# KC-decoder/Multimodal-Brain-Pattern-Identification_XAI

Hardware: AMD Instinct MI355X
Metric: samples/sec train (multimodal SpectrogramCNN+EEGNet fusion, B=64/GPU, 4x128x256 spectro + 10000x19 EEG) (higher is better)
Workload: dtype bf16

## Files before the change

include/brainxai.h:

```cpp
#ifndef BRAINXAI_H
#define BRAINXAI_H

#include <stddef.h>
#include <stdint.h>

#ifdef __cplusplus
extern "C" {
#endif

#define BX_VERSION 100

enum { BX_F32 = 0, BX_BF16 = 1 };
enum { BX_POOL_MAX = 0, BX_POOL_AVG = 1 };
enum { BX_OK = 0, BX_EINVAL = -1, BX_EDTYPE = -2, BX_EALIGN = -3, BX_EWORKSPACE = -4, BX_EHIP = -5,
       BX_EUNSUPPORTED = -6 };
enum { BX_ALGO_AUTO = 0, BX_ALGO_DIRECT = 1, BX_ALGO_MFMA = 2 };
enum { BX_EPI_RELU = 1, BX_EPI_MASK_BITS = 2 };

typedef void* bxStream;

int bx_version(void);
const char* bx_last_error_string(void);

int bx_nchw_to_nhwc(const float* src, void* dst, int B, int C, int H, int W, int Cp, int dtype, bxStream stream);
// ... 35 lines not shown
} bxWgradPending;
int bx_conv3x3_wgrad_chained(const void* x, const void* dz, float* dw_oihw, float* dbias, int B, int H, int W, int Cin,
                             int Ci_p, int Co, int dtype, int algo, void* workspace, size_t workspace_bytes,
                             bxWgradPending* pending, bxStream stream);
int bx_conv3x3_wgrad_finish(bxWgradPending* pending, bxStream stream);
int bx_conv3x3_carry(const void* x, const float* packed_f32, const void* packed_mfma, const float* bias,
                     const void* relu_mask_src, const void* addend, void* y, int B, int H, int W, int Ci, int Co,
                     int dtype, int flags, int algo, bxWgradPending* pending, bxStream stream);
int bx_conv3x3_carry_many(const void* x, const float* packed_f32, const void* packed_mfma, const float* bias,
                          const void* relu_mask_src, const void* addend, void* y, int B, int H, int W, int Ci, int Co,
                          int dtype, int flags, int algo, bxWgradPending* pending, int npending, bxStream stream);
typedef struct {
  const void* x; const void* dz;
  float* dw; float* db;
  int Cin, Ci_p, Co;
} bxWgradGroupLayer;
int bx_conv3x3_wgrad_group_supported(int n, const int* Ci_p, const int* Co, int W, int dtype);
size_t bx_conv3x3_wgrad_group_workspace(const bxWgradGroupLayer* layers, int n, int B, int H, int W, int dtype);
int bx_conv3x3_wgrad_group(const bxWgradGroupLayer* layers, int n, int B, int H, int W, int dtype, void* workspace,
                           size_t workspace_bytes, bxWgradPending* pending, bxStream stream);
size_t bx_conv3x3_bwd_fused_workspace(int B, int H, int W, int with_w1);
int bx_conv3x3_bwd_fused(const void* dz, const void* xl, const void* packed_flip, void* dzo, const void* x0, float* dw, float* db,
                         float* dw0, float* db0, int B, int H, int W, int Cin0, void* workspace, size_t workspace_bytes,
                         bxWgradPending* pending, bxStream stream);

int bx_profile_next_conv3(void* ev_start, void* ev_stop);

typedef struct {
  int B, H, W;
  int Cin_p;
  int C;
  int pool;
  int training;
  float eps, momentum;
  float dropout_p;
  uint32_t salt;
  int dtype;
  uint32_t* sync;
  void* route;
  int pool_h, pool_w;
} bxTailDesc;
size_t bx_block_tail_route_bytes(const bxTailDesc* d);
#define BX_TAIL_SYNC_WORDS 8192
#define BX_TAIL_SYNC_FWD 0
#define BX_TAIL_SYNC_BWD 4096
size_t bx_block_tail_workspace(const bxTailDesc* d);
int bx_block_tail_fwd(const bxTailDesc* d, const void* y3, const void* x, const float* w1x1, int Cin,
                      const float* b1x1, const float* bn_weight, const float* bn_bias,
                      float* running_mean, float* running_var, int64_t* num_batches_tracked,
                      const uint64_t* seed, void* pooled, void* out, float* save_mean, float* save_invstd,
                      void* workspace, size_t workspace_bytes, bxStream stream);
int bx_set_tree_max_rows(int rows);
int bx_set_tail_fold(int mask);
int bx_block_conv3_tail_fwd(const bxTailDesc* d, const void* y2, const void* w3_mfma, const float* b3, void* y3,
                            const void* x, const float* w1x1, int Cin, const float* b1x1, const float* bn_weight,
                            const float* bn_bias, float* running_mean, float* running_var, int64_t* num_batches_tracked,
                            const uint64_t* seed, void* pooled, void* out, float* save_mean, float* save_invstd,
                            void* workspace, size_t workspace_bytes, bxStream stream);
int bx_block_tail_bwd(const bxTailDesc* d, const void* dout, const void* y3, const void* x, const void* pooled,
                      const float* w1x1, int Cin, const float* bn_weight, const float* save_mean,
                      const float* save_invstd, const uint64_t* seed, void* dz3, void* dx_skip,
                      float* d_bn_weight, float* d_bn_bias, float* d_w1x1, float* d_b1x1,
                      void* workspace, size_t workspace_bytes, bxStream stream);
int bx_relu(const void* x, void* y, size_t n, int dtype, bxStream stream);

int bx_gap_fc_lsm_fwd(const void* feat, const float* w, const float* b, float* gap_out, float* logp,
                      int B, int HW, int C, int N, int dtype, bxStream stream);
int bx_gap_fc_lsm_bwd(const float* dlogp, const float* logp, const float* gap_out, const float* w,
                      void* dfeat, float* dw, float* db, int B, int HW, int C, int N, int dtype, bxStream stream);
int bx_linear_lsm_fwd(const float* x, const float* w, const float* b, float* logp, int B, int K, int N,
                      bxStream stream);
int bx_linear_lsm_bwd(const float* dlogp, const float* logp, const float* x, const float* w, float* dx,
                      float* dw, float* db, int B, int K, int N, bxStream stream);
int bx_fusion_head_fwd(const float* eeg_logp, const float* spec_logp, const float* w1, const float* b1,
                       const float* w2, const float* b2, float* hidden, float* logp, int B, int N, int Hd,
                       bxStream stream);
int bx_fusion_head_bwd(const float* dlogp, const float* logp, const float* hidden, const float* eeg_logp,
                       const float* spec_logp, const float* w1, const float* w2, float* d_eeg_logp,
                       float* d_spec_logp, float* dw1, float* db1, float* dw2, float* db2, int B, int N, int Hd,
                       bxStream stream);
size_t bx_mm_head_workspace(int B, int N, int Hd);
int bx_mm_head_fwd(const void* feat, const float* eeg_feat, const float* fc_w, const float* fc_b, const float* dense_w,
                   const float* dense_b, const float* w1, const float* b1, const float* w2, const float* b2,
                   float* gap_out, float* spec_logp, float* eeg_logp, float* hidden, float* logp, int B, int HW, int C,
                   int K, int N, int Hd, int dtype, bxStream stream);
int bx_mm_head_bwd(const float* dlogp, const float* logp, const float* hidden, const float* spec_logp,
                   const float* eeg_logp, const float* gap, const float* eeg_feat, const float* fc_w,
                   const float* dense_w, const float* w1, const float* w2, void* dfeat, float* d_eeg_feat,
                   float* d_fc_w, float* d_fc_b, float* d_dense_w, float* d_dense_b, float* dw1, float* db1, float* dw2,
                   float* db2, void* workspace, size_t workspace_bytes, int B, int HW, int C, int K, int N, int Hd,
                   int dtype, bxStream stream);
int bx_kldiv_fwd_bwd(const float* logp, const float* target, float* loss, float* dlogp, int B, int N,
                     int reduction, float grad_scale, bxStream stream);

typedef struct {
  int B, Chans, T;
  int F1, D, F2;
  int K1, K2;
  int P1, P2;
  int training;
  float eps, momentum, dropout_p;
  uint32_t salt;
  int dtype;
  int collapse;
  float dropout_p2;
  const float* const* x_slot;
// ... 190 lines not shown
```

multimodal-brain-pattern-identification_xai_amd/_lib.py:

```python
from __future__ import annotations

import ctypes as C
import os

HERE = os.path.dirname(os.path.abspath(__file__))
LIB_PATH = os.path.join(HERE, "libbrainxai.so")

BX_F32, BX_BF16 = 0, 1
BX_POOL_MAX, BX_POOL_AVG = 0, 1
BX_ALGO_AUTO, BX_ALGO_DIRECT, BX_ALGO_MFMA = 0, 1, 2
BX_EPI_RELU = 1
BX_EPI_MASK_BITS = 2
BX_TAIL_SYNC_WORDS = 8192
BX_EEG_CAM_CONV1, BX_EEG_CAM_DEPTHWISE, BX_EEG_CAM_SEPARABLE = 0, 1, 2
BX_CAM_GRADCAM, BX_CAM_GRADCAM_PP, BX_CAM_LAYERCAM = 0, 1, 2
BX_SCORECAM_PROB, BX_SCORECAM_INCREASE = 0, 1

vp, i32, i64, u32, f32, sz = C.c_void_p, C.c_int, C.c_int64, C.c_uint32, C.c_float, C.c_size_t


class TailDesc(C.Structure):
    _fields_ = [("B", i32), ("H", i32), ("W", i32), ("Cin_p", i32), ("C", i32), ("pool", i32), ("training", i32),
                ("eps", f32), ("momentum", f32), ("dropout_p", f32), ("salt", u32), ("dtype", i32), ("sync", vp), ("route", vp),
                ("pool_h", i32), ("pool_w", i32)]
# ... 26 lines not shown

class WgradPending(C.Structure):
    _fields_ = [("partial", vp), ("dw", vp), ("db", vp), ("nsplit", i32), ("Cin", i32), ("Co", i32), ("ma", i32), ("nb", i32),
                ("ztiles", i32), ("nfrag4", i32), ("valid", i32)]


class WgradGroupLayer(C.Structure):
    _fields_ = [("x", vp), ("dz", vp), ("dw", vp), ("db", vp), ("Cin", i32), ("Ci_p", i32), ("Co", i32)]


class PackJob(C.Structure):
    _fields_ = [("w_oihw", vp), ("packed_mfma", vp), ("Cout", i32), ("Cin", i32), ("I_p", i32), ("O_p", i32),
                ("transpose_flip", i32), ("block_begin", i32)]


class EegGrads(C.Structure):
    _fields_ = [(n, vp) for n in ("conv1_w", "bn1_w", "bn1_b", "dw_w", "bn2_w", "bn2_b", "sep_w", "bn3_w", "bn3_b")]


P = C.POINTER
SIGNATURES = {
    "bx_version": (i32, []),
    "bx_last_error_string": (C.c_char_p, []),
    "bx_nchw_to_nhwc": (i32, [vp, vp, i32, i32, i32, i32, i32, i32, vp]),
    "bx_nhwc_to_nchw": (i32, [vp, vp, i32, i32, i32, i32, i32, i32, vp]),
    "bx_conv3x3_pack": (i32, [vp, vp, vp, i32, i32, i32, i32, i32, vp]),
    "bx_conv3x3_packed_mfma_bytes": (sz, [i32, i32]),
    "bx_conv3x3_packed_split_bytes": (sz, [i32, i32]),
    "bx_conv3x3_pack_split": (i32, [vp, vp, i32, i32, i32, i32, i32, vp]),
    "bx_conv3x3_pack_many": (i32, [vp, i32, i32, vp]),
    "bx_conv3x3_pack_many_layout": (i32, [vp, i32, i32, vp, vp, i32, i32, i32, i32, i32, vp]),
    "bx_conv3x3_pack_layout_ex": (i32, [vp, i32, i32, vp, vp, vp, i32, i32, i32, i32, i32, vp]),
    "bx_conv3x3_pair_supported": (i32, [i32, i32, i32, i32]),
    "bx_conv3x3_pair": (i32, [vp] * 9 + [i32] * 7 + [vp]),
    "bx_conv3x3_pack_many_step": (i32, [vp, i32, i32, vp, vp, i32, i32, i32, i32, i32, vp, vp, vp, vp, vp]),
    "bx_scale_dev": (i32, [vp, vp, vp, sz, vp]),
    "bx_abs": (i32, [vp, vp, sz, vp]),
    "bx_conv3x3": (i32, [vp, vp, vp, vp, vp, vp, vp, i32, i32, i32, i32, i32, i32, i32, i32, vp]),
    "bx_conv3x3_carry": (i32, [vp, vp, vp, vp, vp, vp, vp, i32, i32, i32, i32, i32, i32, i32, i32, P(WgradPending), vp]),
    "bx_conv3x3_carry_many": (i32, [vp, vp, vp, vp, vp, vp, vp, i32, i32, i32, i32, i32, i32, i32, i32, P(WgradPending), i32, vp]),
    "bx_conv3x3_wgrad_group_supported": (i32, [i32, P(i32), P(i32), i32, i32]),
    "bx_conv3x3_wgrad_group_workspace": (sz, [P(WgradGroupLayer), i32, i32, i32, i32, i32]),
    "bx_conv3x3_wgrad_group": (i32, [P(WgradGroupLayer), i32, i32, i32, i32, i32, vp, sz, P(WgradPending), vp]),
    "bx_conv3x3_wgrad_workspace": (sz, [i32, i32, i32, i32, i32, i32, i32]),
    "bx_conv3x3_wgrad": (i32, [vp, vp, vp, vp, i32, i32, i32, i32, i32, i32, i32, i32, vp, sz, vp]),
    "bx_conv3x3_wgrad_chained": (i32, [vp, vp, vp, vp, i32, i32, i32, i32, i32, i32, i32, i32, vp, sz, P(WgradPending), vp]),
    "bx_conv3x3_wgrad_finish": (i32, [P(WgradPending), vp]),
    "bx_conv3x3_bwd_fused_workspace": (sz, [i32, i32, i32, i32]),
    "bx_conv3x3_bwd_fused": (i32, [vp] * 9 + [i32] * 4 + [vp, sz, P(WgradPending), vp]),
    "bx_block_tail_workspace": (sz, [P(TailDesc)]),
    "bx_block_tail_fwd": (i32, [P(TailDesc), vp, vp, vp, i32, vp, vp, vp, vp, vp, vp, vp, vp, vp, vp, vp, vp, sz, vp]),
    "bx_set_tree_max_rows": (i32, [i32]),
    "bx_set_tail_fold": (i32, [i32]),
    "bx_block_tail_route_bytes": (sz, [vp]),
    "bx_block_conv3_tail_fwd": (i32, [P(TailDesc), vp, vp, vp, vp, vp, vp, i32, vp, vp, vp, vp, vp, vp, vp, vp, vp, vp, vp, vp, sz, vp]),
    "bx_block_tail_bwd": (i32, [P(TailDesc), vp, vp, vp, vp, vp, i32, vp, vp, vp, vp, vp, vp, vp, vp, vp, vp, vp, sz, vp]),
    "bx_relu": (i32, [vp, vp, sz, i32, vp]),
    "bx_gap_fc_lsm_fwd": (i32, [vp, vp, vp, vp, vp, i32, i32, i32, i32, i32, vp]),
    "bx_gap_fc_lsm_bwd": (i32, [vp, vp, vp, vp, vp, vp, vp, i32, i32, i32, i32, i32, vp]),
    "bx_linear_lsm_fwd": (i32, [vp, vp, vp, vp, i32, i32, i32, vp]),
    "bx_linear_lsm_bwd": (i32, [vp, vp, vp, vp, vp, vp, vp, i32, i32, i32, vp]),
    "bx_fusion_head_fwd": (i32, [vp, vp, vp, vp, vp, vp, vp, vp, i32, i32, i32, vp]),
    "bx_fusion_head_bwd": (i32, [vp] * 13 + [i32, i32, i32, vp]),
    "bx_mm_head_workspace": (sz, [i32, i32, i32]),
    "bx_mm_head_fwd": (i32, [vp] * 15 + [i32] * 7 + [vp]),
    "bx_mm_head_bwd": (i32, [vp] * 22 + [sz] + [i32] * 7 + [vp]),
    "bx_kldiv_fwd_bwd": (i32, [vp, vp, vp, vp, i32, i32, i32, f32, vp]),
    "bx_eeg_saved_bytes": (sz, [P(EegDesc)]),
    "bx_eeg_workspace": (sz, [P(EegDesc)]),
    "bx_eeg_features_fwd": (i32, [P(EegDesc), P(EegParams), vp, vp, vp, vp, vp, sz, vp]),
    "bx_eeg_features_bwd": (i32, [P(EegDesc), P(EegParams), vp, vp, vp, vp, P(EegGrads), vp, vp, sz, vp]),
    "bx_eeg_saved_layout": (i32, [P(EegDesc), P(sz), P(sz)]),
    "bx_eeg_gradcam_workspace": (sz, [P(EegDesc), i32, i32]),
    "bx_eeg_gradcam": (i32, [P(EegDesc), P(EegParams), vp, vp, vp, i32, i32, i32, vp, vp, vp, vp, sz, vp]),
    "bx_eeg_cam_workspace": (sz, [P(EegDesc), i32, i32, i32]),
    "bx_eeg_cam": (i32, [P(EegDesc), P(EegParams), vp, vp, vp, i32, i32, i32, i32, vp, vp, vp, vp, sz, vp]),
    "bx_eeg_deep_saved_bytes": (sz, [P(EegDeepDesc)]),
    "bx_eeg_deep_workspace": (sz, [P(EegDeepDesc)]),
    "bx_eeg_deep_fwd": (i32, [P(EegDeepDesc), P(EegDeepParams), vp, vp, vp, vp, vp, vp, sz, vp]),
    "bx_eeg_deep_bwd": (i32, [P(EegDeepDesc), P(EegDeepParams), vp, vp, vp, vp, vp, P(EegDeepGrads), vp, vp, sz, vp]),
    "bx_attention_workspace": (sz, [i32]),
    "bx_attention_fwd": (i32, [vp] * 10 + [i32, i32, i32, vp]),
    "bx_attention_bwd": (i32, [vp] * 16 + [sz, i32, i32, i32, vp]),
    "bx_gradcam_reduce": (i32, [vp, vp, vp, vp, i32, i32, i32, i32, i32, i32, vp]),
    "bx_gradcam_head": (i32, [vp] * 12 + [i32] * 8 + [vp]),
    "bx_gradcam_head_sweep": (i32, [vp] * 4 + [i32] + [vp] * 8 + [i32] * 11 + [vp]),
    "bx_cam_reduce": (i32, [vp, vp, vp, vp, i32, i32, i32, i32, i32, i32, i32, vp]),
    "bx_cam_head": (i32, [vp] * 12 + [i32] * 9 + [vp]),
    "bx_cam_head_sweep": (i32, [vp] * 4 + [i32] + [vp] * 8 + [i32] * 12 + [vp]),
    "bx_resize_bilinear": (i32, [vp, vp, i32, i32, i32, i32, i32, vp]),
    "bx_saliency_reduce": (i32, [vp, vp, i32, i32, i32, i32, f32, i32, vp]),
    "bx_axpby": (i32, [vp, vp, sz, f32, f32, vp]),
    "bx_mul": (i32, [vp, vp, vp, sz, vp]),
    "bx_ig_interpolate": (i32, [vp, vp, vp, vp, sz, i32, vp]),
    "bx_ig_accumulate": (i32, [vp, vp, vp, sz, i32, vp]),
    "bx_eeg_stack_iir": (i32, [vp, vp, vp, i32, i32, i32, i32, P(C.c_double), P(C.c_double), i32, i32, f32, f32, vp]),
    "bx_eeg_montage_workspace": (sz, [i32, i32, i32, i32]),
    "bx_eeg_montage_stack": (i32, [vp, vp, vp, vp, i32, i32, i32, i32, i32, P(C.c_double), P(C.c_double), i32, P(C.c_double), P(C.c_double),
                                   i32, f32, vp, vp, sz, vp]),
    "bx_spec_preprocess_workspace": (sz, [i32, i32, i32]),
    "bx_spec_preprocess": (i32, [vp, vp, vp, i32, i32, i32, i32, i32, i32, P(C.c_double), P(C.c_double), P(C.c_double), P(C.c_double),
                                 f32, vp, vp, sz, vp]),
    "bx_spec_regions_workspace": (sz, [i32]),
    "bx_spec_regions": (i32, [vp, vp, vp] + [i32] * 7 + [P(C.c_double), i32, P(C.c_double), i32, f32, vp, sz, vp]),
    "bx_adamw_step": (i32, [vp, vp, vp, vp, sz, f32, f32, f32, f32, f32, f32, vp, vp]),
    "bx_adamw_partials": (sz, [sz]),
# ... 66 lines not shown
```

multimodal-brain-pattern-identification_xai_amd/csrc/tail.hip:

```cpp
#include "bx_common.h"

#define TAIL_MAX_GROUPS 128
#define TAIL_MAX_BLOCKS 2048

struct TailGeom {
  int B, H, W, Ho, Wo, C, Cin_p, ncg, slots;
  long long npool;
  float sy, sx;
};

static int tail_ph(const bxTailDesc* d) { return d->pool_h ? d->pool_h : 2; }
static int tail_pw(const bxTailDesc* d) { return d->pool_w ? d->pool_w : 2; }
static bool tail_2x2(const bxTailDesc* d) { return tail_ph(d) == 2 && tail_pw(d) == 2; }

static int make_geom(const bxTailDesc* d, TailGeom* g) {
  if (tail_ph(d) < 1 || tail_pw(d) < 1) return -5;
  g->B = d->B; g->H = d->H; g->W = d->W; g->Ho = d->H / tail_ph(d); g->Wo = d->W / tail_pw(d); g->C = d->C; g->Cin_p = d->Cin_p;
  if (d->B <= 0 || g->Ho <= 0 || g->Wo <= 0) return -1;
  if (d->C % 8 || d->C > 256 || 256 % (d->C / 8)) return -2;
  if (d->Cin_p % 8 || d->Cin_p <= 0) return -3;
  if ((long long)d->B * d->H * d->W * ((d->Cin_p > d->C ? d->Cin_p : d->C) / 8) >= (1ll << 31)) return -4;
  g->ncg = d->C / 8; g->slots = 256 / g->ncg;
  g->npool = (long long)d->B * g->Ho * g->Wo;
  g->sy = (float)d->H / (float)g->Ho; g->sx = (float)d->W / (float)g->Wo;
// ... 151 lines not shown
        ld8(y3, base + ((size_t)r * g.W + (q - r * pw)) * g.C, w[u]);
      }
#pragma unroll
      for (int u = 0; u < 4; ++u)
        if (q0 + u < area)
#pragma unroll
          for (int j = 0; j < 8; ++j) v[j] = pool == BX_POOL_MAX ? fmaxf(v[j], w[u][j]) : v[j] + w[u][j];
    }
    if (pool != BX_POOL_MAX)
#pragma unroll
      for (int j = 0; j < 8; ++j) v[j] = v[j] / (float)area;
    st8(pooled, (size_t)pp * g.C + cg * 8, v);
    if (want_stats) {
#pragma unroll
      for (int j = 0; j < 8; ++j) {
        const float q = round_as(pooled, v[j]);
        acc[0][j] += q; acc[1][j] += q * q;
      }
    }
  }
  if (!want_stats) return;
  pool_stats_publish(acc, lds, partials, g, tree, fin);
}

template <typename T> struct Raw8;
template <> struct Raw8<bf16_t> {
  uint4 r;
  __device__ __forceinline__ void load(const bf16_t* p, size_t i) { r = *reinterpret_cast<const uint4*>(p + i); }
  __device__ __forceinline__ void get(float v[8]) const {
    const uint32_t w[4] = {r.x, r.y, r.z, r.w};
#pragma unroll
    for (int k = 0; k < 4; ++k) { v[2 * k] = __uint_as_float(w[k] << 16); v[2 * k + 1] = __uint_as_float(w[k] & 0xffff0000u); }
  }
};
template <> struct Raw8<float> {
  float4 a, b;
  __device__ __forceinline__ void load(const float* p, size_t i) { a = *reinterpret_cast<const float4*>(p + i); b = *reinterpret_cast<const float4*>(p + i + 4); }
  __device__ __forceinline__ void get(float v[8]) const { v[0] = a.x; v[1] = a.y; v[2] = a.z; v[3] = a.w; v[4] = b.x; v[5] = b.y; v[6] = b.z; v[7] = b.w; }
};

template <typename T>
__device__ __forceinline__ void skip_sample(const T* __restrict__ x, const TailGeom& g, int b, int oy, int ox, int c0, float out[8]) {
  int y0, y1, x0, x1; float ly, lx;
  bilinear_src(oy, g.sy, g.H, y0, y1, ly);
  bilinear_src(ox, g.sx, g.W, x0, x1, lx);
  const float hy = 1.f - ly, hx = 1.f - lx;
  float p00[8], p01[8], p10[8], p11[8];
  const size_t rb = (size_t)b * g.H;
  ld8(x, ((rb + y0) * g.W + x0) * g.Cin_p + c0, p00); ld8(x, ((rb + y0) * g.W + x1) * g.Cin_p + c0, p01);
  ld8(x, ((rb + y1) * g.W + x0) * g.Cin_p + c0, p10); ld8(x, ((rb + y1) * g.W + x1) * g.Cin_p + c0, p11);
#pragma unroll
  for (int j = 0; j < 8; ++j) out[j] = hy * (hx * p00[j] + lx * p01[j]) + ly * (hx * p10[j] + lx * p11[j]);
}

struct TailFwdPro { const float* rows; int nrows; BxBnFinalize fin; };
template <typename T, int RPT>
__global__ __launch_bounds__(256, sizeof(T) == 4 ? 3 : 4) void k_tail_apply(const T* __restrict__ pooled, const T* __restrict__ x, const float* __restrict__ wT,
    int Cin, const float* __restrict__ b1x1, const float* __restrict__ scale, const float* __restrict__ shift,
    const uint64_t* __restrict__ seed, float dropout_p, uint32_t salt, T* __restrict__ out, TailGeom g,
    const float* __restrict__ ev_gamma, const float* __restrict__ ev_beta, const float* __restrict__ ev_rmean,
    const float* __restrict__ ev_rvar, float eps, float* __restrict__ save_mean, float* __restrict__ save_invstd, TailFwdPro pro) {
  extern __shared__ float xs[];
  const int cg = threadIdx.x % g.ncg, slot = threadIdx.x / g.ncg;
  const int xstride = g.Cin_p + 1, nci8 = g.Cin_p / 8;
  const uint64_t sd = (dropout_p > 0.f && seed) ? seed[0] : 0;
  const float inv_keep = dropout_p > 0.f ? 1.f / (1.f - dropout_p) : 1.f;
  float sc[8], sh[8], bb[8];
  if (pro.rows) {
    __shared__ __attribute__((aligned(8))) double sp[BX_ROWS_TOTAL_LDS(2) / 8];
    __shared__ float ssc[2][256];
    bx_rows_total<2>(pro.rows, pro.nrows, g.C, sp);
    if ((int)threadIdx.x < g.C) {
      const int c = threadIdx.x;
      const BxBnFinalize& f = pro.fin;
      float mean, invstd; double unbiased;
      bx_bn_batch_stats(sp[c], sp[g.C + c], f.count, f.eps, mean, invstd, unbiased);
      const float s_ = f.gamma[c] * invstd, h_ = f.beta[c] - mean * s_;
      ssc[0][c] = s_; ssc[1][c] = h_;
      if (blockIdx.x == 0) {
        f.rmean[c] = (1.f - f.momentum) * f.rmean[c] + f.momentum * mean;
        f.rvar[c] = (1.f - f.momentum) * f.rvar[c] + f.momentum * (float)unbiased;
        if (c == 0 && f.nbt) f.nbt[0] += 1;
        f.scale[c] = s_; f.shift[c] = h_; f.save_mean[c] = mean; f.save_invstd[c] = invstd;
      }
    }
    __syncthreads();
#pragma unroll
    for (int j = 0; j < 8; ++j) { sc[j] = ssc[0][cg * 8 + j]; sh[j] = ssc[1][cg * 8 + j]; bb[j] = b1x1[cg * 8 + j]; }
  } else if (ev_gamma) {
#pragma unroll
    for (int j = 0; j < 8; ++j) {
      const int c = cg * 8 + j;
      const float is = 1.0f / sqrtf(ev_rvar[c] + eps), s_ = ev_gamma[c] * is;
      sc[j] = s_; sh[j] = ev_beta[c] - ev_rmean[c] * s_; bb[j] = b1x1[c];
    }
    if (blockIdx.x == 0 && (int)threadIdx.x < g.C) {
      save_mean[threadIdx.x] = ev_rmean[threadIdx.x];
      save_invstd[threadIdx.x] = 1.0f / sqrtf(ev_rvar[threadIdx.x] + eps);
    }
  } else {
#pragma unroll
    for (int j = 0; j < 8; ++j) { sc[j] = scale[cg * 8 + j]; sh[j] = shift[cg * 8 + j]; bb[j] = b1x1[cg * 8 + j]; }
  }
  const long long nsteps = (g.npool + (long long)gridDim.x * g.slots - 1) / ((long long)gridDim.x * g.slots);
  for (long long st = 0; st < nsteps; ++st) {
    const long long p0 = (st * gridDim.x + blockIdx.x) * g.slots;
    Raw8<T> pvr;
    {
      const long long ppq = p0 + slot;
      pvr.load(pooled, (size_t)(ppq < g.npool ? ppq : 0) * g.C + cg * 8);
    }
    __syncthreads();
    for (int u = threadIdx.x; u < g.slots * nci8; u += 256) {
      const int sl = u / nci8, c8 = u % nci8;
      const long long pp = p0 + sl;
      if (pp < g.npool) {
        int ox, oy, b;
        px_decode(pp, g.Wo, g.Ho, ox, oy, b);
        float v[8];
        skip_sample(x, g, b, oy, ox, c8 * 8, v);
#pragma unroll
        for (int j = 0; j < 8; ++j) xs[sl * xstride + c8 * 8 + j] = v[j];
      }
    }
    __syncthreads();
    const long long pp = p0 + slot;
    if (pp >= g.npool) continue;
    float pv[8], acc[8];
    pvr.get(pv);
#pragma unroll
    for (int j = 0; j < 8; ++j) {
      float v = pv[j] * sc[j] + sh[j];
      if (dropout_p > 0.f) v *= bx_dropout_scale(sd, salt, (uint64_t)pp * g.C + cg * 8 + j, dropout_p, inv_keep);
      acc[j] = v + bb[j];
    }
    constexpr int H = RPT / 4;
    float4 wa[2][H], wb[2][H];
    auto load_rows = [&](int c0, float4 (&a)[H], float4 (&b)[H]) {
#pragma unroll
      for (int u = 0; u < H; ++u) {
        a[u] = *reinterpret_cast<const float4*>(wT + (size_t)(c0 + u) * g.C + cg * 8);
        b[u] = *reinterpret_cast<const float4*>(wT + (size_t)(c0 + u) * g.C + cg * 8 + 4);
      }
    };
    auto use_rows = [&](int c0, const float4 (&a)[H], const float4 (&b)[H]) {
#pragma unroll
      for (int u = 0; u < H; ++u) {
        const float xv = xs[slot * xstride + c0 + u];
        acc[0] = fmaf(a[u].x, xv, acc[0]); acc[1] = fmaf(a[u].y, xv, acc[1]); acc[2] = fmaf(a[u].z, xv, acc[2]); acc[3] = fmaf(a[u].w, xv, acc[3]);
        acc[4] = fmaf(b[u].x, xv, acc[4]); acc[5] = fmaf(b[u].y, xv, acc[5]); acc[6] = fmaf(b[u].z, xv, acc[6]); acc[7] = fmaf(b[u].w, xv, acc[7]);
      }
    };
    load_rows(0, wa[0], wb[0]);
    for (int c0 = 0; c0 < g.Cin_p; c0 += 2 * H) {
      load_rows(c0 + H, wa[1], wb[1]);
      use_rows(c0, wa[0], wb[0]);
      if (c0 + 2 * H < g.Cin_p) load_rows(c0 + 2 * H, wa[0], wb[0]);
      use_rows(c0 + H, wa[1], wb[1]);
    }
    st8(out, (size_t)pp * g.C + cg * 8, acc);
  }
}

static int g_tree_max_rows = -1;
int bx_tree_max_rows() {
  if (g_tree_max_rows < 0) { const char* e = getenv("BX_TREE_MAX_ROWS"); g_tree_max_rows = e ? atoi(e) : 0; }
  return g_tree_max_rows;
}
extern "C" int bx_set_tree_max_rows(int rows) {
  BX_REQUIRE(rows >= 0, "bx_set_tree_max_rows: rows must be >= 0");
  g_tree_max_rows = rows;
  return BX_OK;
}
static int g_tail_fold = -1;
static int tail_fold() {
  if (g_tail_fold < 0) { const char* e = getenv("BX_TAIL_FOLD"); g_tail_fold = e ? atoi(e) & 3 : 3; }
  return g_tail_fold;
}
int bx_tail_fold_mask() { return tail_fold(); }
extern "C" int bx_set_tail_fold(int mask) {
  BX_REQUIRE(mask >= 0 && mask <= 3, "bx_set_tail_fold: mask is a combination of 1 (backward) and 2 (forward)");
  g_tail_fold = mask;
  return BX_OK;
}
constexpr int TAIL_FOLD_RC_BWD = 8192;
constexpr int TAIL_FOLD_RC_FWD = 32768;
constexpr int TAIL_FOLD_GRID = 512;
static bool tail_fold_ok(const TailGeom& g) { return g.C <= 256 && bx_rows_total_ok(g.C); }
static int tail_fold_rows(int C) { const int r = TAIL_FOLD_RC_BWD / C; return r < 16 ? 16 : r > TAIL_MAX_BLOCKS ? TAIL_MAX_BLOCKS : r; }
static size_t tail_rows_cap(const bxTailDesc* d) {
  const size_t conv_rows = (size_t)d->B * ((d->H + 7) / 8) * ((d->W + 15) / 16);
  return conv_rows > TAIL_MAX_BLOCKS ? conv_rows : TAIL_MAX_BLOCKS;
}
extern "C" size_t bx_block_tail_route_bytes(const bxTailDesc* d) {
  TailGeom g;
  if (!d || make_geom(d, &g) || !tail_2x2(d)) return 0;
  return (size_t)g.npool * g.C / 2;
}
extern "C" size_t bx_block_tail_workspace(const bxTailDesc* d) {
  TailGeom g;
  if (!d || make_geom(d, &g)) return 0;
  const size_t Ho = g.Ho, Wo = g.Wo;
  size_t fwd = ((size_t)tail_rows_cap(d) * 2 + 2) * d->C * sizeof(float) + (size_t)d->Cin_p * d->C * sizeof(float)
             + (size_t)TAIL_MAX_GROUPS * 2 * d->C * sizeof(double);
  size_t bwd = ((size_t)TAIL_MAX_BLOCKS * 3 + 3) * d->C * sizeof(float)
             + bx_align_up((size_t)d->B * Ho * Wo * d->Cin_p * sizeof(float), 256)
             + (size_t)2048 * 256 * sizeof(float) + (size_t)65 * d->C * d->Cin_p * sizeof(float);
  return bx_align_up(fwd > bwd ? fwd : bwd, 256) + (size_t)TAIL_MAX_GROUPS * 3 * d->C * sizeof(double);
}

extern "C" int bx_block_tail_fwd(const bxTailDesc* d, const void* y3, const void* x, const float* w1x1, int Cin,
                                 const float* b1x1, const float* bn_weight, const float* bn_bias,
                                 float* running_mean, float* running_var, int64_t* num_batches_tracked,
                                 const uint64_t* seed, void* pooled, void* out, float* save_mean, float* save_invstd,
                                 void* workspace, size_t workspace_bytes, bxStream stream) {
  BX_REQUIRE(d && y3 && x && w1x1 && b1x1 && bn_weight && bn_bias && running_mean && running_var && pooled && out && save_mean && save_invstd,
             "bx_block_tail_fwd: null pointer");
  BX_DTYPE_OK(d->dtype);
  TailGeom g;
  const int ge = make_geom(d, &g);
  BX_REQUIRE(ge == 0, "bx_block_tail_fwd: unsupported geometry (code %d): need C%%8==0, C<=256, 256%%(C/8)==0, Cin_p%%8==0, "
             "pool_h, pool_w >= 0, H >= pool_h, W >= pool_w", ge);
  BX_REQUIRE(Cin > 0 && Cin <= d->Cin_p, "bx_block_tail_fwd: Cin=%d exceeds Cin_p=%d", Cin, d->Cin_p);
  BX_REQUIRE(d->dropout_p >= 0.f && d->dropout_p < 1.f, "bx_block_tail_fwd: dropout_p must be in [0,1)");
  BX_REQUIRE(d->dropout_p == 0.f || !d->training || seed, "bx_block_tail_fwd: dropout needs a device seed");
  const size_t need = bx_block_tail_workspace(d);
  if (!workspace || workspace_bytes < need) BX_FAIL(BX_EWORKSPACE, "bx_block_tail_fwd: workspace %zu < %zu", workspace_bytes, need);
  const size_t xs_bytes = (size_t)g.slots * (g.Cin_p + 1) * sizeof(float);
  BX_REQUIRE(xs_bytes <= 60 * 1024, "bx_block_tail_fwd: Cin_p too large for the LDS tile");
  hipStream_t s = (hipStream_t)stream;
  const int nblk = tail_blocks(g);
  float* partials = (float*)workspace;
  float* scale = partials + tail_rows_cap(d) * 2 * g.C;
  float* shift = scale + g.C;
  float* wT = shift + g.C;
  const float p = d->training ? d->dropout_p : 0.f;
  const bool in_launch = d->training && d->sync && 256 % g.C == 0 && nblk <= bx_tree_max_rows();
  BxStatTree tree = {};
  BxBnFinalize fin = {};
  if (in_launch) {
    tree.rows = partials; tree.cnt = d->sync + BX_TAIL_SYNC_FWD; tree.nrows = nblk; tree.Cw = tree.ld = g.C;
    bx_stat_tree_shape(nblk, &tree.G, &tree.ngroups);
    tree.mid = (double*)(wT + (size_t)g.Cin_p * g.C);
    BX_REQUIRE(tree.ngroups + 1 <= BX_TAIL_SYNC_BWD - BX_TAIL_SYNC_FWD, "bx_block_tail_fwd: %d reduction groups exceed the sync block", tree.ngroups);
    fin = BxBnFinalize{bn_weight, bn_bias, running_mean, running_var, num_batches_tracked, d->momentum, d->eps, scale, shift, save_mean, save_invstd,
                       (double)g.npool};
  }
  if (tail_2x2(d)) {
    BX_DISPATCH_DTYPE(d->dtype, T,
      hipLaunchKernelGGL((k_pool_stats<T>), dim3(nblk), dim3(256), 0, s, (const T*)y3, (T*)pooled, partials, g, d->pool, d->training,
                         w1x1, Cin, wT, tree, fin));
  } else {
    BX_DISPATCH_DTYPE(d->dtype, T,
      hipLaunchKernelGGL((k_pool_stats_win<T>), dim3(nblk), dim3(256), 0, s, (const T*)y3, (T*)pooled, partials, g, tail_ph(d), tail_pw(d),
                         d->pool, d->training, w1x1, Cin, wT, tree, fin));
  }
  BX_CHECK_LAUNCH("bx_block_tail_fwd(pool)");
  const bool fold = d->training && !in_launch && (tail_fold() & 2) && tail_fold_ok(g) && (long long)nblk * g.C <= TAIL_FOLD_RC_FWD;
  TailFwdPro pro = {};
  if (fold)
    pro = TailFwdPro{partials, nblk, BxBnFinalize{bn_weight, bn_bias, running_mean, running_var, num_batches_tracked, d->momentum, d->eps, scale, shift,
                                                 save_mean, save_invstd, (double)g.npool}};
  if (d->training && !in_launch && !fold) {
    hipLaunchKernelGGL(k_bn_finalize, dim3(bx_finalize_grid(g.C)), dim3(1024), 0, s, partials, nblk, (double)g.npool, g.C, d->training, bn_weight, bn_bias,
                       running_mean, running_var, num_batches_tracked, d->momentum, d->eps, scale, shift, save_mean, save_invstd);
    BX_CHECK_LAUNCH("bx_block_tail_fwd(finalize)");
  }
  const bool ev = !d->training;
  const int napply = fold && tail_blocks_all(g) > TAIL_FOLD_GRID ? TAIL_FOLD_GRID : tail_blocks_all(g);
  BX_DISPATCH_DTYPE(d->dtype, T,
    hipLaunchKernelGGL((k_tail_apply<T, 8>), dim3(napply), dim3(256), xs_bytes, s, (const T*)pooled, (const T*)x, wT, Cin, b1x1,
                       scale, shift, seed, p, d->salt, (T*)out, g, ev ? bn_weight : (const float*)nullptr, bn_bias, (const float*)running_mean,
                       (const float*)running_var, d->eps, save_mean, save_invstd, pro));
  BX_CHECK_LAUNCH("bx_block_tail_fwd(apply)");
  return BX_OK;
}

extern "C" int bx_block_conv3_tail_fwd(const bxTailDesc* d, const void* y2, const void* w3_mfma, const float* b3, void* y3,
                                       const void* x, const float* w1x1, int Cin, const float* b1x1, const float* bn_weight, const float* bn_bias,
                                       float* running_mean, float* running_var, int64_t* num_batches_tracked,
                                       const uint64_t* seed, void* pooled, void* out, float* save_mean, float* save_invstd,
                                       void* workspace, size_t workspace_bytes, bxStream stream) {
  BX_REQUIRE(d && y2 && w3_mfma && b3 && x && w1x1 && b1x1 && bn_weight && bn_bias && running_mean && running_var && pooled && out && save_mean
             && save_invstd, "bx_block_conv3_tail_fwd: null pointer");
  if (d->dtype != BX_BF16 || !bx_conv3x3_mfma_supported(d->C, d->C, d->dtype) || d->C < 16)
    BX_FAIL(BX_EUNSUPPORTED, "bx_block_conv3_tail_fwd: needs bf16 storage and an MFMA-capable channel count (C=%d dtype=%d)", d->C, d->dtype);
  if (!tail_2x2(d))
    BX_FAIL(BX_EUNSUPPORTED, "bx_block_conv3_tail_fwd: the fused epilogue pools 2x2 windows only (pool %dx%d)", tail_ph(d), tail_pw(d));
  TailGeom g;
  const int ge = make_geom(d, &g);
  BX_REQUIRE(ge == 0, "bx_block_conv3_tail_fwd: unsupported geometry (code %d)", ge);
  BX_REQUIRE(Cin > 0 && Cin <= d->Cin_p, "bx_block_conv3_tail_fwd: Cin=%d exceeds Cin_p=%d", Cin, d->Cin_p);
  BX_REQUIRE(d->dropout_p >= 0.f && d->dropout_p < 1.f, "bx_block_conv3_tail_fwd: dropout_p must be in [0,1)");
  BX_REQUIRE(d->dropout_p == 0.f || !d->training || seed, "bx_block_conv3_tail_fwd: dropout needs a device seed");
  const size_t need = bx_block_tail_workspace(d);
  if (!workspace || workspace_bytes < need) BX_FAIL(BX_EWORKSPACE, "bx_block_conv3_tail_fwd: workspace %zu < %zu", workspace_bytes, need);
  const size_t xs_bytes = (size_t)g.slots * (g.Cin_p + 1) * sizeof(float);
  BX_REQUIRE(xs_bytes <= 60 * 1024, "bx_block_conv3_tail_fwd: Cin_p too large for the LDS tile");
  hipStream_t s = (hipStream_t)stream;
  float* partials = (float*)workspace;
  float* scale = partials + tail_rows_cap(d) * 2 * g.C;
  float* shift = scale + g.C;
  float* wT = shift + g.C;
  BxConvPoolEpi pe = {};
  pe.pooled = pooled; pe.pool = d->pool; pe.want_stats = d->training; pe.Ho = g.Ho; pe.Wo = g.Wo;
  pe.w1x1 = w1x1; pe.wT = wT; pe.Cin1 = Cin; pe.Cin1_p = g.Cin_p;
  pe.route = d->route; pe.route_bytes = (uint32_t)bx_block_tail_route_bytes(d); pe.store_y = y3 != nullptr;
  if (d->training) {
    pe.tree.rows = partials; pe.tree.mid = (double*)(wT + (size_t)g.Cin_p * g.C); pe.tree.cnt = d->sync ? d->sync + BX_TAIL_SYNC_FWD : nullptr;
    pe.rows_cap_floats = tail_rows_cap(d) * 2 * g.C; pe.cnt_cap_words = BX_TAIL_SYNC_BWD - BX_TAIL_SYNC_FWD; pe.tree_max_rows = bx_tree_max_rows();
    pe.fin = BxBnFinalize{bn_weight, bn_bias, running_mean, running_var, num_batches_tracked, d->momentum, d->eps, scale, shift, save_mean, save_invstd,
                          (double)g.npool};
  }
  if (g_bx_prof_ev[0]) (void)hipEventRecord(g_bx_prof_ev[0], s);
  const int rc = bx_conv3x3_mfma_pool_launch(y2, w3_mfma, b3, y3, d->B, d->H, d->W, d->C, d->C, &pe, s);
  if (g_bx_prof_ev[1]) (void)hipEventRecord(g_bx_prof_ev[1], s);
  g_bx_prof_ev[0] = g_bx_prof_ev[1] = nullptr;
  if (rc != BX_OK) return rc;
  const bool fold = d->training && !pe.tree.cnt && (tail_fold() & 2) && tail_fold_ok(g) && (long long)pe.tree.nrows * g.C <= TAIL_FOLD_RC_FWD
                    && pe.tree.nrows <= 1024;
  TailFwdPro pro = {};
  if (fold) pro = TailFwdPro{partials, pe.tree.nrows, pe.fin};
  if (d->training && !pe.tree.cnt && !fold) {
    hipLaunchKernelGGL(k_bn_finalize, dim3(bx_finalize_grid(g.C)), dim3(1024), 0, s, partials, pe.tree.nrows, (double)g.npool, g.C, 1, bn_weight, bn_bias,
                       running_mean, running_var, num_batches_tracked, d->momentum, d->eps, scale, shift, save_mean, save_invstd);
    BX_CHECK_LAUNCH("bx_block_conv3_tail_fwd(finalize)");
  }
  const float p = d->training ? d->dropout_p : 0.f;
  const bool ev = !d->training;
  const int napply = fold && tail_blocks_all(g) > TAIL_FOLD_GRID ? TAIL_FOLD_GRID : tail_blocks_all(g);
  hipLaunchKernelGGL((k_tail_apply<bf16_t, 8>), dim3(napply), dim3(256), xs_bytes, s, (const bf16_t*)pooled, (const bf16_t*)x, wT, Cin, b1x1,
                     scale, shift, seed, p, d->salt, (bf16_t*)out, g, ev ? bn_weight : (const float*)nullptr, bn_bias, (const float*)running_mean,
                     (const float*)running_var, d->eps, save_mean, save_invstd, pro);
  BX_CHECK_LAUNCH("bx_block_conv3_tail_fwd(apply)");
  return BX_OK;
}

struct TailBwdFin { const float* gamma; const float* invstd; float* coef; float* dgamma; float* dbeta; float* db1x1; double count; int training; };
__device__ __forceinline__ void tail_bwd_finalize_channel(int c, int C, const double (&s)[3], const TailBwdFin& f) {
  if (f.dbeta) f.dbeta[c] = (float)s[0];
  if (f.dgamma) f.dgamma[c] = (float)s[1];
  if (f.db1x1) f.db1x1[c] = (float)s[2];
  f.coef[c] = f.gamma[c] * f.invstd[c];
  f.coef[C + c] = f.training ? (float)(s[0] / f.count) : 0.f;
  f.coef[2 * C + c] = f.training ? (float)(s[1] / f.count) : 0.f;
}
template <typename T, int NPT = 2>
__device__ __forceinline__ void tail_bwd_reduce_body(const T* __restrict__ dout, const T* __restrict__ pooled,
    const float* __restrict__ mean, const float* __restrict__ invstd, const uint64_t* __restrict__ seed, float dropout_p,
    uint32_t salt, float* partials, const TailGeom& g, int bid, int nblocks, const BxStatTree& tree, const TailBwdFin& fin) {
  __shared__ __attribute__((aligned(16))) float lds[2048];
  const int cg = threadIdx.x % g.ncg, slot = threadIdx.x / g.ncg;
  const uint64_t sd = (dropout_p > 0.f && seed) ? seed[0] : 0;
  const float inv_keep = dropout_p > 0.f ? 1.f / (1.f - dropout_p) : 1.f;
  float mu[8], is[8], acc[3][8];
#pragma unroll
  for (int j = 0; j < 8; ++j) { mu[j] = mean[cg * 8 + j]; is[j] = invstd[cg * 8 + j]; acc[0][j] = acc[1][j] = acc[2][j] = 0.f; }
  const long long stride = (long long)nblocks * g.slots;
  for (long long pp0 = (long long)bid * g.slots + slot; pp0 < g.npool; pp0 += NPT * stride) {
    float go[NPT][8], pv[NPT][8];
    bool ok[NPT];
#pragma unroll
    for (int h = 0; h < NPT; ++h) {
      const long long pp = pp0 + h * stride;
      ok[h] = pp < g.npool;
      if (ok[h]) { ld8(dout, (size_t)pp * g.C + cg * 8, go[h]); ld8(pooled, (size_t)pp * g.C + cg * 8, pv[h]); }
    }
#pragma unroll
    for (int h = 0; h < NPT; ++h) {
      if (!ok[h]) continue;
      const long long pp = pp0 + h * stride;
#pragma unroll
      for (int j = 0; j < 8; ++j) {
        float dd = go[h][j];
        if (dropout_p > 0.f) dd *= bx_dropout_scale(sd, salt, (uint64_t)pp * g.C + cg * 8 + j, dropout_p, inv_keep);
        acc[0][j] += dd;
        acc[1][j] += dd * (pv[h][j] - mu[j]) * is[j];
        acc[2][j] += go[h][j];
      }
    }
  }
  float red[3];
  block_channel_reduce<3>(acc, lds, g.C, g.ncg, g.slots, red);
  if (tree.cnt) {
    double tot[3];
    __syncthreads();
// ... 736 lines not shown
```

Baseline: 49580.

## Add persistent streaming tail-apply kernel with register-prefetched loads for small channel counts

Adds a persistent-grid kernel, k_tail_apply_stream, for the residual block tail (BN apply, dropout, bias plus bilinear-resampled 1x1 skip conv) when Cin_p is 8 or 16 and C is at most 64. It keeps the 1x1 weights and the BN coefficients in LDS, prefetches the next pixel's pooled and skip-corner loads into registers while computing the current one, and broadcasts input channels across lanes with DPP. The grid is capped at the resident-block count from an occupancy query. This targets latency-bound memory access in the generic apply kernel for the small-channel early blocks, at the cost of more register pressure and a second code path that can be selected through an environment variable.

```diff
diff --git a/include/brainxai.h b/include/brainxai.h
--- a/include/brainxai.h
+++ b/include/brainxai.h
@@ -111,6 +111,8 @@
                       void* workspace, size_t workspace_bytes, bxStream stream);
 int bx_set_tree_max_rows(int rows);
 int bx_set_tail_fold(int mask);
+int bx_set_tail_stream(int n);
+int bx_tail_stream_applies(int Cin_p, int C, int dtype);
 int bx_block_conv3_tail_fwd(const bxTailDesc* d, const void* y2, const void* w3_mfma, const float* b3, void* y3,
                             const void* x, const float* w1x1, int Cin, const float* b1x1, const float* bn_weight,
                             const float* bn_bias, float* running_mean, float* running_var, int64_t* num_batches_tracked,
diff --git a/multimodal-brain-pattern-identification_xai_amd/_lib.py b/multimodal-brain-pattern-identification_xai_amd/_lib.py
--- a/multimodal-brain-pattern-identification_xai_amd/_lib.py
+++ b/multimodal-brain-pattern-identification_xai_amd/_lib.py
@@ -102,6 +102,8 @@
     "bx_block_tail_fwd": (i32, [P(TailDesc), vp, vp, vp, i32, vp, vp, vp, vp, vp, vp, vp, vp, vp, vp, vp, vp, sz, vp]),
     "bx_set_tree_max_rows": (i32, [i32]),
     "bx_set_tail_fold": (i32, [i32]),
+    "bx_set_tail_stream": (i32, [i32]),
+    "bx_tail_stream_applies": (i32, [i32, i32, i32]),
     "bx_block_tail_route_bytes": (sz, [vp]),
     "bx_block_conv3_tail_fwd": (i32, [P(TailDesc), vp, vp, vp, vp, vp, vp, i32, vp, vp, vp, vp, vp, vp, vp, vp, vp, vp, vp, vp, sz, vp]),
     "bx_block_tail_bwd": (i32, [P(TailDesc), vp, vp, vp, vp, vp, i32, vp, vp, vp, vp, vp, vp, vp, vp, vp, vp, vp, sz, vp]),
diff --git a/multimodal-brain-pattern-identification_xai_amd/csrc/tail.hip b/multimodal-brain-pattern-identification_xai_amd/csrc/tail.hip
--- a/multimodal-brain-pattern-identification_xai_amd/csrc/tail.hip
+++ b/multimodal-brain-pattern-identification_xai_amd/csrc/tail.hip
@@ -227,20 +227,40 @@
 #pragma unroll
   for (int j = 0; j < 8; ++j) out[j] = hy * (hx * p00[j] + lx * p01[j]) + ly * (hx * p10[j] + lx * p11[j]);
 }
+__device__ __forceinline__ void skip_corners(const TailGeom& g, int b, int oy, int ox, int c0, size_t off[4], float& ly, float& lx) {
+  int y0, y1, x0, x1;
+  bilinear_src(oy, g.sy, g.H, y0, y1, ly);
+  bilinear_src(ox, g.sx, g.W, x0, x1, lx);
+  const size_t rb = (size_t)b * g.H;
+  off[0] = ((rb + y0) * g.W + x0) * g.Cin_p + c0; off[1] = ((rb + y0) * g.W + x1) * g.Cin_p + c0;
+  off[2] = ((rb + y1) * g.W + x0) * g.Cin_p + c0; off[3] = ((rb + y1) * g.W + x1) * g.Cin_p + c0;
+}
+template <typename T>
+__device__ __forceinline__ void skip_blend(const float p00[8], const float p01[8], const float p10[8], const float p11[8], float ly, float lx, float out[8]) {
+  const float hy = 1.f - ly, hx = 1.f - lx;
+#pragma unroll
+  for (int j = 0; j < 8; ++j) {
+    const float top = (sizeof(T) == 2 || j < 3) ? fmaf(p01[j], lx, p00[j] * hx) : fmaf(p00[j], hx, lx * p01[j]);
+    const float bot = fmaf(hx, p10[j], lx * p11[j]);
+    out[j] = fmaf(hy, top, ly * bot);
+  }
+}
+template <bool DROP>
+__device__ __forceinline__ float tail_bn_drop_bias(float pv, float sc, float sh, float bb, float keep) {
+  float v = fmaf(pv, sc, sh);
+  if (DROP) { v = v * keep; asm("" : "+v"(v)); }
+  return v + bb;
+}
 
 struct TailFwdPro { const float* rows; int nrows; BxBnFinalize fin; };
-template <typename T, int RPT>
-__global__ __launch_bounds__(256, sizeof(T) == 4 ? 3 : 4) void k_tail_apply(const T* __restrict__ pooled, const T* __restrict__ x, const float* __restrict__ wT,
-    int Cin, const float* __restrict__ b1x1, const float* __restrict__ scale, const float* __restrict__ shift,
-    const uint64_t* __restrict__ seed, float dropout_p, uint32_t salt, T* __restrict__ out, TailGeom g,
-    const float* __restrict__ ev_gamma, const float* __restrict__ ev_beta, const float* __restrict__ ev_rmean,
-    const float* __restrict__ ev_rvar, float eps, float* __restrict__ save_mean, float* __restrict__ save_invstd, TailFwdPro pro) {
-  extern __shared__ float xs[];
-  const int cg = threadIdx.x % g.ncg, slot = threadIdx.x / g.ncg;
-  const int xstride = g.Cin_p + 1, nci8 = g.Cin_p / 8;
-  const uint64_t sd = (dropout_p > 0.f && seed) ? seed[0] : 0;
-  const float inv_keep = dropout_p > 0.f ? 1.f / (1.f - dropout_p) : 1.f;
-  float sc[8], sh[8], bb[8];
+struct TailFwdCoef {
+  const float* b1x1; const float* scale; const float* shift;
+  const float* ev_gamma; const float* ev_beta; const float* ev_rmean; const float* ev_rvar; float eps; float* save_mean; float* save_invstd;
+};
+__device__ __forceinline__ void tail_fwd_coefs(const TailGeom& g, int cg, const TailFwdCoef& k, const TailFwdPro& pro, float sc[8], float sh[8], float bb[8]) {
+  const float* __restrict__ b1x1 = k.b1x1; const float* __restrict__ scale = k.scale; const float* __restrict__ shift = k.shift;
+  const float* __restrict__ ev_gamma = k.ev_gamma; const float* __restrict__ ev_beta = k.ev_beta; const float* __restrict__ ev_rmean = k.ev_rmean;
+  const float* __restrict__ ev_rvar = k.ev_rvar; const float eps = k.eps; float* __restrict__ save_mean = k.save_mean; float* __restrict__ save_invstd = k.save_invstd;
   if (pro.rows) {
     __shared__ __attribute__((aligned(8))) double sp[BX_ROWS_TOTAL_LDS(2) / 8];
     __shared__ float ssc[2][256];
@@ -277,6 +297,21 @@
 #pragma unroll
     for (int j = 0; j < 8; ++j) { sc[j] = scale[cg * 8 + j]; sh[j] = shift[cg * 8 + j]; bb[j] = b1x1[cg * 8 + j]; }
   }
+}
+
+template <typename T, int RPT>
+__global__ __launch_bounds__(256, sizeof(T) == 4 ? 3 : 4) void k_tail_apply(const T* __restrict__ pooled, const T* __restrict__ x, const float* __restrict__ wT,
+    int Cin, const float* __restrict__ b1x1, const float* __restrict__ scale, const float* __restrict__ shift,
+    const uint64_t* __restrict__ seed, float dropout_p, uint32_t salt, T* __restrict__ out, TailGeom g,
+    const float* __restrict__ ev_gamma, const float* __restrict__ ev_beta, const float* __restrict__ ev_rmean,
+    const float* __restrict__ ev_rvar, float eps, float* __restrict__ save_mean, float* __restrict__ save_invstd, TailFwdPro pro) {
+  extern __shared__ float xs[];
+  const int cg = threadIdx.x % g.ncg, slot = threadIdx.x / g.ncg;
+  const int xstride = g.Cin_p + 1, nci8 = g.Cin_p / 8;
+  const uint64_t sd = (dropout_p > 0.f && seed) ? seed[0] : 0;
+  const float inv_keep = dropout_p > 0.f ? 1.f / (1.f - dropout_p) : 1.f;
+  float sc[8], sh[8], bb[8];
+  tail_fwd_coefs(g, cg, TailFwdCoef{b1x1, scale, shift, ev_gamma, ev_beta, ev_rmean, ev_rvar, eps, save_mean, save_invstd}, pro, sc, sh, bb);
   const long long nsteps = (g.npool + (long long)gridDim.x * g.slots - 1) / ((long long)gridDim.x * g.slots);
   for (long long st = 0; st < nsteps; ++st) {
     const long long p0 = (st * gridDim.x + blockIdx.x) * g.slots;
@@ -337,6 +372,105 @@
   }
 }
 
+constexpr int TAIL_STREAM_MAX_C = 64;
+template <int K> __device__ __forceinline__ float quad_bcast(float v) { return bx_dpp<K * 0x55>(v); }
+template <typename T, int NCH, int NPX>
+struct TailStreamTrip {
+  Raw8<T> pv[NPX], cr[NPX][4];
+  float ly[NPX], lx[NPX];
+  __device__ __forceinline__ void issue(const T* __restrict__ pooled, const T* __restrict__ x, const TailGeom& g, long long base, long long stride, int slot, int cg) {
+#pragma unroll
+    for (int h = 0; h < NPX; ++h) {
+      const long long pq = base + h * stride + slot;
+      const unsigned pp = (unsigned)(pq < g.npool ? pq : g.npool - 1);
+      int ox, oy, b;
+      px_decode(pp, g.Wo, g.Ho, ox, oy, b);
+      size_t off[4];
+      skip_corners(g, b, oy, ox, (cg % NCH) * 8, off, ly[h], lx[h]);
+      pv[h].load(pooled, (size_t)(pp * (unsigned)g.ncg + (unsigned)cg) * 8);
+#pragma unroll
+      for (int q = 0; q < 4; ++q) cr[h][q].load(x, off[q]);
+    }
+  }
+};
+template <int K, int NCH, int NPX>
+__device__ __forceinline__ void tail_stream_rows(const float* wl, int C, int woff, const float (&xv)[NPX][8], float (&acc)[NPX][8]) {
+  float4 wa[2], wb[2];
+  wa[0] = *reinterpret_cast<const float4*>(wl + woff + K * 8 * C); wb[0] = *reinterpret_cast<const float4*>(wl + woff + K * 8 * C + 4);
+#pragma unroll
+  for (int j = 0; j < 8; ++j) {
+    if (j < 7) {
+      const float* w = wl + woff + (K * 8 + j + 1) * C;
+      wa[(j + 1) & 1] = *reinterpret_cast<const float4*>(w); wb[(j + 1) & 1] = *reinterpret_cast<const float4*>(w + 4);
+    }
+    const float4 a = wa[j & 1], b = wb[j & 1];
+#pragma unroll
+    for (int h = 0; h < NPX; ++h) {
+      const float xs = NCH > 1 ? quad_bcast<K>(xv[h][j]) : xv[h][j];
+      acc[h][0] = fmaf(a.x, xs, acc[h][0]); acc[h][1] = fmaf(a.y, xs, acc[h][1]); acc[h][2] = fmaf(a.z, xs, acc[h][2]); acc[h][3] = fmaf(a.w, xs, acc[h][3]);
+      acc[h][4] = fmaf(b.x, xs, acc[h][4]); acc[h][5] = fmaf(b.y, xs, acc[h][5]); acc[h][6] = fmaf(b.z, xs, acc[h][6]); acc[h][7] = fmaf(b.w, xs, acc[h][7]);
+    }
+#pragma unroll
+    for (int h = 0; h < NPX; ++h)
+      asm volatile("" : "+v"(woff), "+v"(acc[h][0]), "+v"(acc[h][1]), "+v"(acc[h][2]), "+v"(acc[h][3]), "+v"(acc[h][4]), "+v"(acc[h][5]),
+                        "+v"(acc[h][6]), "+v"(acc[h][7]));
+  }
+}
+template <typename T, int NCH, int NPX, bool DROP>
+__global__ __launch_bounds__(256, 4) void k_tail_apply_stream(const T* __restrict__ pooled, const T* __restrict__ x,
+    const float* __restrict__ wT, const uint64_t* __restrict__ seed, float dropout_p, uint32_t salt, T* __restrict__ out, TailGeom g,
+    TailFwdCoef coef, TailFwdPro pro) {
+  __shared__ __attribute__((aligned(16))) float wl[NCH * 8 * TAIL_STREAM_MAX_C];
+  __shared__ __attribute__((aligned(16))) float cl[3][TAIL_STREAM_MAX_C];
+  const int cg = threadIdx.x % g.ncg, slot = threadIdx.x / g.ncg;
+  const uint64_t sd = (DROP && seed) ? seed[0] : 0;
+  const float inv_keep = DROP ? 1.f / (1.f - dropout_p) : 1.f;
+  const long long stride = (long long)gridDim.x * g.slots;
+  long long base = (long long)blockIdx.x * g.slots;
+  TailStreamTrip<T, NCH, NPX> t;
+  if (base < g.npool) t.issue(pooled, x, g, base, stride, slot, cg);
+  lds_fill<4>(wl, NCH * 8 * g.C, [&](int k) { return wT[k]; });
+  {
+    float sc[8], sh[8], bb[8];
+    tail_fwd_coefs(g, cg, coef, pro, sc, sh, bb);
+    if (slot == 0) {
+#pragma unroll
+      for (int j = 0; j < 8; ++j) { cl[0][cg * 8 + j] = sc[j]; cl[1][cg * 8 + j] = sh[j]; cl[2][cg * 8 + j] = bb[j]; }
+    }
+  }
+  __syncthreads();
+  while (base < g.npool) {
+    asm volatile("" ::: "memory");
+    float xv[NPX][8], acc[NPX][8];
+#pragma unroll
+    for (int h = 0; h < NPX; ++h) {
+      float p00[8], p01[8], p10[8], p11[8];
+      t.cr[h][0].get(p00); t.cr[h][1].get(p01); t.cr[h][2].get(p10); t.cr[h][3].get(p11);
+      skip_blend<T>(p00, p01, p10, p11, t.ly[h], t.lx[h], xv[h]);
+    }
+    float sc[8], sh[8], bb[8];
+    ld8(cl[0], cg * 8, sc); ld8(cl[1], cg * 8, sh); ld8(cl[2], cg * 8, bb);
+#pragma unroll
+    for (int h = 0; h < NPX; ++h) {
+      float pvf[8];
+      t.pv[h].get(pvf);
+      const uint64_t e0 = (uint64_t)(base + h * stride + slot) * g.C + cg * 8;
+#pragma unroll
+      for (int j = 0; j < 8; ++j)
+        acc[h][j] = tail_bn_drop_bias<DROP>(pvf[j], sc[j], sh[j], bb[j], DROP ? bx_dropout_scale(sd, salt, e0 + j, dropout_p, inv_keep) : 1.f);
+    }
+    tail_stream_rows<0, NCH, NPX>(wl, g.C, cg * 8, xv, acc);
+    if constexpr (NCH > 1) tail_stream_rows<1, NCH, NPX>(wl, g.C, cg * 8, xv, acc);
+#pragma unroll
+    for (int h = 0; h < NPX; ++h) {
+      const long long pq = base + h * stride + slot;
+      if (pq < g.npool) st8(out, (size_t)((unsigned)pq * (unsigned)g.ncg + (unsigned)cg) * 8, acc[h]);
+    }
+    base += NPX * stride;
+    if (base < g.npool) t.issue(pooled, x, g, base, stride, slot, cg);
+  }
+}
+
 static int g_tree_max_rows = -1;
 int bx_tree_max_rows() {
   if (g_tree_max_rows < 0) { const char* e = getenv("BX_TREE_MAX_ROWS"); g_tree_max_rows = e ? atoi(e) : 0; }
@@ -362,6 +496,72 @@
 constexpr int TAIL_FOLD_RC_FWD = 32768;
 constexpr int TAIL_FOLD_GRID = 512;
 static bool tail_fold_ok(const TailGeom& g) { return g.C <= 256 && bx_rows_total_ok(g.C); }
+constexpr int TAIL_STREAM_UNSET = -2;
+static int g_tail_stream = TAIL_STREAM_UNSET;
+static int tail_stream() {
+  if (g_tail_stream == TAIL_STREAM_UNSET) { const char* e = getenv("BX_TAIL_STREAM"); const int v = e ? atoi(e) : -1; g_tail_stream = v < -1 ? -1 : v; }
+  return g_tail_stream;
+}
+extern "C" int bx_set_tail_stream(int n) {
+  BX_REQUIRE(n >= -1, "bx_set_tail_stream: -1 (shape policy), 0 (generic kernel) or a positive workgroup cap");
+  g_tail_stream = n;
+  return BX_OK;
+}
+static bool tail_stream_compiled(int Cin_p, int C) {
+  if (C % 8 || C > TAIL_STREAM_MAX_C || 256 % (C / 8)) return false;
+  return Cin_p == 8 || (Cin_p == 16 && (C / 8) % 4 == 0);
+}
+extern "C" int bx_tail_stream_applies(int Cin_p, int C, int dtype) {
+  if ((dtype != BX_F32 && dtype != BX_BF16) || !tail_stream_compiled(Cin_p, C)) return 0;
+  return tail_stream() != 0;
+}
+template <typename T, bool DROP> constexpr int tail_stream_npx() { return sizeof(T) == 2 && !DROP ? 2 : 1; }
+template <typename T, int NCH, bool DROP>
+static int tail_stream_resident() {
+  static int n = 0;
+  if (n == 0) {
+    int dev = 0, cus = 0, per = 0;
+    if (hipGetDevice(&dev) != hipSuccess || hipDeviceGetAttribute(&cus, hipDeviceAttributeMultiprocessorCount, dev) != hipSuccess
+        || hipOccupancyMaxActiveBlocksPerMultiprocessor(&per, k_tail_apply_stream<T, NCH, tail_stream_npx<T, DROP>(), DROP>, 256, 0) != hipSuccess
+        || cus <= 0 || per <= 0)
+      return -1;
+    n = cus * per;
+  }
+  return n;
+}
+struct TailApplyArgs {
+  const void* pooled; const void* x; const float* wT; int Cin; const uint64_t* seed; float dropout_p; uint32_t salt; void* out;
+  TailFwdCoef coef; TailFwdPro pro;
+};
+template <typename T, int NCH, bool DROP>
+static int tail_apply_stream_launch(const TailGeom& g, const TailApplyArgs& a, int cap, hipStream_t s) {
+  constexpr int NPX = tail_stream_npx<T, DROP>();
+  const int resident = tail_stream_resident<T, NCH, DROP>();
+  BX_REQUIRE(resident > 0, "block tail: the occupancy query for the streaming apply kernel failed");
+  long long grid = (g.npool + (long long)g.slots * NPX - 1) / ((long long)g.slots * NPX);
+  if (grid > resident) grid = resident;
+  if (cap > 0 && grid > cap) grid = cap;
+  hipLaunchKernelGGL((k_tail_apply_stream<T, NCH, NPX, DROP>), dim3((unsigned)grid), dim3(256), 0, s, (const T*)a.pooled, (const T*)a.x, a.wT, a.seed,
+                     a.dropout_p, a.salt, (T*)a.out, g, a.coef, a.pro);
+  return BX_OK;
+}
+template <typename T, int NCH>
+static int tail_apply_stream_launch(const TailGeom& g, const TailApplyArgs& a, int cap, hipStream_t s) {
+  return a.dropout_p > 0.f ? tail_apply_stream_launch<T, NCH, true>(g, a, cap, s) : tail_apply_stream_launch<T, NCH, false>(g, a, cap, s);
+}
+template <typename T>
+static int tail_apply_launch(const TailGeom& g, int dtype, const TailApplyArgs& a, hipStream_t s) {
+  if (bx_tail_stream_applies(g.Cin_p, g.C, dtype)) {
+    const int cap = tail_stream();
+    return g.Cin_p == 8 ? tail_apply_stream_launch<T, 1>(g, a, cap, s) : tail_apply_stream_launch<T, 2>(g, a, cap, s);
+  }
+  const size_t xs_bytes = (size_t)g.slots * (g.Cin_p + 1) * sizeof(float);
+  const int napply = a.pro.rows && tail_blocks_all(g) > TAIL_FOLD_GRID ? TAIL_FOLD_GRID : tail_blocks_all(g);
+  const TailFwdCoef& k = a.coef;
+  hipLaunchKernelGGL((k_tail_apply<T, 8>), dim3(napply), dim3(256), xs_bytes, s, (const T*)a.pooled, (const T*)a.x, a.wT, a.Cin, k.b1x1, k.scale, k.shift,
+                     a.seed, a.dropout_p, a.salt, (T*)a.out, g, k.ev_gamma, k.ev_beta, k.ev_rmean, k.ev_rvar, k.eps, k.save_mean, k.save_invstd, a.pro);
+  return BX_OK;
+}
 static int tail_fold_rows(int C) { const int r = TAIL_FOLD_RC_BWD / C; return r < 16 ? 16 : r > TAIL_MAX_BLOCKS ? TAIL_MAX_BLOCKS : r; }
 static size_t tail_rows_cap(const bxTailDesc* d) {
   const size_t conv_rows = (size_t)d->B * ((d->H + 7) / 8) * ((d->W + 15) / 16);
@@ -442,11 +642,11 @@
     BX_CHECK_LAUNCH("bx_block_tail_fwd(finalize)");
   }
   const bool ev = !d->training;
-  const int napply = fold && tail_blocks_all(g) > TAIL_FOLD_GRID ? TAIL_FOLD_GRID : tail_blocks_all(g);
-  BX_DISPATCH_DTYPE(d->dtype, T,
-    hipLaunchKernelGGL((k_tail_apply<T, 8>), dim3(napply), dim3(256), xs_bytes, s, (const T*)pooled, (const T*)x, wT, Cin, b1x1,
-                       scale, shift, seed, p, d->salt, (T*)out, g, ev ? bn_weight : (const float*)nullptr, bn_bias, (const float*)running_mean,
-                       (const float*)running_var, d->eps, save_mean, save_invstd, pro));
+  const TailApplyArgs aa = {pooled, x, wT, Cin, seed, p, d->salt, out,
+                            TailFwdCoef{b1x1, scale, shift, ev ? bn_weight : nullptr, bn_bias, running_mean, running_var, d->eps, save_mean, save_invstd}, pro};
+  int rc = BX_OK;
+  BX_DISPATCH_DTYPE(d->dtype, T, rc = tail_apply_launch<T>(g, d->dtype, aa, s));
+  if (rc != BX_OK) return rc;
   BX_CHECK_LAUNCH("bx_block_tail_fwd(apply)");
   return BX_OK;
 }
@@ -503,10 +703,10 @@
   }
   const float p = d->training ? d->dropout_p : 0.f;
   const bool ev = !d->training;
-  const int napply = fold && tail_blocks_all(g) > TAIL_FOLD_GRID ? TAIL_FOLD_GRID : tail_blocks_all(g);
-  hipLaunchKernelGGL((k_tail_apply<bf16_t, 8>), dim3(napply), dim3(256), xs_bytes, s, (const bf16_t*)pooled, (const bf16_t*)x, wT, Cin, b1x1,
-                     scale, shift, seed, p, d->salt, (bf16_t*)out, g, ev ? bn_weight : (const float*)nullptr, bn_bias, (const float*)running_mean,
-                     (const float*)running_var, d->eps, save_mean, save_invstd, pro);
+  const TailApplyArgs aa = {pooled, x, wT, Cin, seed, p, d->salt, out,
+                            TailFwdCoef{b1x1, scale, shift, ev ? bn_weight : nullptr, bn_bias, running_mean, running_var, d->eps, save_mean, save_invstd}, pro};
+  const int arc = tail_apply_launch<bf16_t>(g, d->dtype, aa, s);
+  if (arc != BX_OK) return arc;
   BX_CHECK_LAUNCH("bx_block_conv3_tail_fwd(apply)");
   return BX_OK;
 }
```

Result: no change. 49800 (median of 6 runs) (+0.4%).
